# gillesdegottex/percivaltts

Hardware: AMD Instinct MI355X
Metric: acoustic frames/sec per WGAN-GP critic+gen step (higher is better)
Workload: dtype f32

## Files before the change

include/percival_hip.h:

```cpp
#ifndef PERCIVAL_HIP_H
#define PERCIVAL_HIP_H

#include <stddef.h>
#include <stdint.h>

#ifdef __cplusplus
extern "C" {
#endif

#define PTTS_OK            0
#define PTTS_EINVAL       -1
#define PTTS_ELAUNCH      -2
#define PTTS_EWORKSPACE   -3
#define PTTS_EDEVICE      -4

#define PTTS_IN_NONE     0
#define PTTS_IN_LRELU    1
#define PTTS_IN_MASKMUL  2

#define PTTS_PAD_SAME    0
#define PTTS_PAD_CAUSAL  1

#define PTTS_ACT_NONE    0
#define PTTS_ACT_LRELU   1
// ... 79 lines not shown
                          const void* tables, float* partials, size_t partials_bytes, int* nblocks_out, int* npart_out,
                          int B, int T, int F, int L, int cin0, float alpha, void* stream);
int ptts_conv2d_chain_bwd_data(const void* d_last, int d_bf16, const void* maps, const void* a_last, const void* tables,
                               void* gmaps, float* g0, int B, int T, int F, int L, float alpha, void* stream);
int ptts_conv2d_chain_second(const float* u0, const void* gmaps, const void* maps, const void* a_last, const void* tables,
                             void* out, int out_bf16, float* partials, size_t partials_bytes, int* nblocks_out, int* npart_out,
                             int B, int T, int F, int L, int cin0, float alpha, void* stream);

int ptts_gemm(const float* A, const float* Bm, const float* bias, float* C,
              int M, int N, int K,
              int transA, long long lda, long long rows_per_seg, long long seg_stride,
              int transB, long long ldb, long long ldc,
              int in_mode, const float* in_scale, const float* in_shift, const float* mask_src,
              float alpha, int accumulate, const float* out_mask, float* colsum_b, void* stream);

typedef struct ptts_wgrad_desc {
    const float* A; const float* B; float* C; float* colsum_b;
    const float* in_scale; const float* in_shift; const float* mask_src;
    int M, N, K;
    long long lda, ldb, ldc;
    int in_mode; float alpha;
} ptts_wgrad_desc;
int ptts_gemm_wgrad_grouped(const ptts_wgrad_desc* descs, int n, void* stream);

size_t ptts_dense_planes_bytes(int N, int K);
int ptts_split3_dense_weight(const float* w, long long ldw, int K, int N, int transposed, void* planes, void* stream);
typedef struct ptts_dense_split_desc {
    const float* w; void* planes;
    long long ldw;
    int K, N, transposed, reserved;
} ptts_dense_split_desc;
int ptts_split3_dense_weight_grouped(const ptts_dense_split_desc* descs, int n, void* stream);
int ptts_split3_frame_windows(const float* x, int B, int T, int C, int NS, int S, int row_off, int P, int kvalid,
                              void* planes, long long stride_planes_bytes, void* stream);
int ptts_split3_dense_weight_strided(const float* w, long long stride_w, void* planes, long long stride_planes_bytes, int n,
                                     long long ldw, int K, int N, int transposed, void* stream);
int ptts_dense_bf16x6_supported(int M, int N, int K, long long lda, long long ldc);
typedef struct ptts_dense_wgrad_reduce_desc {
    const float* partials;
    int split, Kin, N;
    long long ldc;
    float* C; float* colsum_b;
} ptts_dense_wgrad_reduce_desc;
int ptts_dense_wgrad_bf16x6_supported(int Kin, int N, int M, long long lda, long long ldb);
size_t ptts_dense_wgrad_workspace_bytes(int Kin, int N, int M);
int ptts_dense_wgrad_bf16x6_partials(const float* A, const float* dY, const float* mask_src, const float* in_scale,
                                     const float* in_shift, void* workspace, size_t workspace_bytes, int* split_out,
                                     int Kin, int N, int M, long long lda, long long ldb, int in_mode, float alpha,
                                     void* stream);
int ptts_dense_wgrad_reduce_grouped(const ptts_dense_wgrad_reduce_desc* descs, int n, void* stream);
int ptts_dense_wgrad_bf16x6(const float* A, const float* dY, const float* mask_src, const float* in_scale,
                            const float* in_shift, float* C, float* colsum_b, void* workspace, size_t workspace_bytes,
                            int Kin, int N, int M, long long lda, long long ldb, long long ldc, int in_mode, float alpha,
                            void* stream);
int ptts_dense_bf16x6(const float* A, const void* planes, const float* bias, float* C, int M, int N, int K,
                      long long lda, long long ldc, int in_mode, const float* in_scale, const float* in_shift,
                      const float* mask_src, float alpha, int accumulate, const float* out_mask, void* stream);
int ptts_dense_bf16x6_res(const float* A, const void* planes, const float* bias, float* C, int M, int N, int K,
                          long long lda, long long ldc, int in_mode, const float* in_scale, const float* in_shift,
                          const float* mask_src, float alpha, const float* res, int res_rows, long long ldr,
                          const float* out_mask, void* stream);
int ptts_dense_bf16x6_stats_rows(int M, int N);
int ptts_dense_bf16x6_stats(const float* A, const void* planes, const float* bias, float* C, int M, int N, int K,
                            long long lda, long long ldc, int in_mode, const float* in_scale, const float* in_shift,
                            float alpha, double* stats, int capacity_rows, int* nrows_out, void* stream);
int ptts_dense_bf16x6_bwd_affine(const float* A, const void* planes, float* C, int M, int N, int K, long long lda, long long ldc,
                                 const float* z, const float* scale, const float* shift, float alpha,
                                 double* stats, int capacity_rows, int* nrows_out, void* stream);
int ptts_partial_rows_sum(const double* partials, int nrows, int ncols, double* out, void* stream);
int ptts_dft_mirror(float* Ap, int NB, int B, int Cin, int Kh, void* stream);

int ptts_conv1d_freq_kernel_planes(const float* w, const float* tw, void* planes, int NB, int KW, int Cin, int N, int Kh, void* stream);

int ptts_transpose_batched(const float* src, float* dst, int nb, int rows, int cols, void* stream);
int ptts_conv1d_freq_wgrad_combine(const float* out2, float* dW, int KW, int Cin, int N, int Kh, void* stream);

size_t ptts_conv1d_freq_wgrad_inverse_workspace_bytes(int KW, int Cin, int N);
int ptts_conv1d_freq_wgrad_inverse(const float* Gt, const float* t2, float* dW, void* workspace, size_t workspace_bytes,
                                   int NB, int NBp, int KW, int Cin, int N, int Kh, void* stream);

int ptts_dense_bf16x6_batched(const float* A, long long strideA, const void* planes, long long stride_planes_bytes,
                              const float* bias, float* C, long long strideC, int nbatch, int M, int N, int K,
                              long long lda, long long ldc, int planes_count, void* stream);
int ptts_dense_tn_bf16x6_batched(const float* A, long long strideA, const float* B, long long strideB, float* C, long long strideC,
                                 int nbatch, int M, int Kin, int N, long long lda, long long ldb, long long ldc, int planes_count,
                                 void* stream);

int ptts_split3_frames(const float* x, void* p1, void* p2, void* p3, int B, int T, int C, int pad_left, int pad_right,
                       int Cp, void* stream);
int ptts_split3_weight_t(const float* w, void* p1, void* p2, void* p3, int KW, int C, int N, int Cp, void* stream);
int ptts_conv1d_bf16x6(const void* a1, const void* a2, const void* a3, const void* bt1, const void* bt2, const void* bt3,
                       const float* bias, float* y, int B, int T, int KW, int Cp, int N, void* stream);

int ptts_split3_frames_t(const float* x, void* p1, void* p2, void* p3, int B, int T, int C, int pad_left, int Tp, int Crows,
                         long long Pp, void* stream);
int ptts_conv1d_wgrad_bf16x6(const void* xt1, const void* xt2, const void* xt3, const void* yt1, const void* yt2,
                             const void* yt3, float* dw, int B, int T, int KW, int C, int N, int Crows, long long Pp,
                             void* stream);

int ptts_transpose_frames(const float* x, float* out, int B, int T, int C, int pad_left, int Tp, int Crows, long long Pp,
                          void* stream);
int ptts_conv1d_wgrad_t(const float* xt, const float* yt, float* dw, float* db, int B, int T, int KW, int C, int N, int Crows,
                        long long Pp, void* stream);

size_t ptts_colstats_workspace_bytes(long long rows, int C);
int ptts_colstats(const float* x, long long rows, int C,
                  int in_mode, const float* in_scale, const float* in_shift, const float* mask_src, float alpha,
                  double* sums , void* workspace, size_t workspace_bytes, void* stream);

int ptts_bn_finalize(const double* sums, long long count, const float* gamma, const float* beta,
                     float* moving_mean, float* moving_var, float eps, float momentum,
                     int training, int update_moving, int unbiased_moving, int C,
                     float* scale, float* shift, float* mean , float* rstd , void* stream);

int ptts_bn_batch_stats_supported(long long rows, int C);
int ptts_bn_batch_stats(const float* x, long long rows, int C, const float* gamma, const float* beta,
                        float* moving_mean, float* moving_var, float eps, float momentum, int update_moving, int unbiased_moving,
                        float* scale, float* shift, float* mean , float* rstd ,
                        void* workspace, size_t workspace_bytes, int* counter, void* stream);

int ptts_bn_finalize_partials(const double* partials, int nrows, long long rows, int C, const float* gamma, const float* beta,
                              float* moving_mean, float* moving_var, float eps, float momentum, int update_moving, int unbiased_moving,
                              float* scale, float* shift, float* mean , float* rstd , void* stream);

int ptts_bn_bwd_coefs(const float* dscale, const float* dshift, const float* mean, const float* rstd,
                      const float* gamma , long long count, int C,
                      float* dgamma, float* dbeta, float* c0, float* c2, void* stream);
int ptts_bn_bwd_coefs_acc(const float* dscale, const float* dshift, const float* mean, const float* rstd,
                      const float* gamma , long long count, int C,
                      float* dgamma, float* dbeta, float* c0, float* c2, void* stream);

int ptts_affine_act(const float* x, const float* scale, const float* shift, float* y,
                    long long rows, int C, int act, float alpha, void* stream);
int ptts_affine_act_bwd(const float* dy, const float* x, const float* y, const float* scale, const float* shift,
                        float* dx, double* dsums ,
                        void* workspace, size_t workspace_bytes,
                        long long rows, int C, int act, float alpha, void* stream);
int ptts_gated_mul_fwd(const float* a, const float* b, float* y, long long n, void* stream);
int ptts_gated_mul_bwd(const float* dy, const float* a, const float* b, float* da, float* db, long long n, void* stream);

int ptts_axpby_cols(const float* a, const float* c1, const float* x, const float* c2, const float* c0,
                    float* out, long long rows, int C, void* stream);

int ptts_gp_interpolate(const float* real, const float* fake, const float* alpha_b , float* out,
                        int B, long long TD, void* stream);
int ptts_gp_sqnorm(const float* g, float* out, int B, long long TD, void* stream);
int ptts_gp_penalty(const float* sq , float* penalty , float* coef , int B, void* stream);
int ptts_gp_scale_rows(const float* g, const float* coef, const float* upstream , float* dg,
                       int B, long long TD, void* stream);

int ptts_mean_scaled(const float* v, long long n, float sign, float* out, void* stream);
int ptts_wlse_fwd(const float* y, const float* yhat, const float* w , float* out,
                  long long rows, int D, void* stream);
int ptts_wlse_bwd(const float* y, const float* yhat, const float* w, const float* upstream, float* dyhat,
                  long long rows, int D, void* stream);

int ptts_weight_clip(float* p, long long n, float lo, float hi, void* stream);

int ptts_adam_keras_step(float* p, const float* g, float* m, float* v, long long n,
                         float lr, float b1, float b2, float eps, float gscale,
                         int* step , void* stream);

size_t ptts_lstm_fwd_workspace_bytes(int B, int T, int H, int ndir);
int ptts_lstm_fwd(const float* xproj, const float* U, float* h_out, float* gates, float* c_out,
                  void* workspace, size_t workspace_bytes,
                  int B, int T, int H, int ndir, int reverse, void* stream);
// ... 113 lines not shown
```

percivaltts_amd/csrc/dense.hip:

```cpp
#include "common.h"
#include <cstdlib>

namespace ptts {
namespace dns {

typedef __bf16 bf16x8 __attribute__((ext_vector_type(8)));
typedef __bf16 bf16x4 __attribute__((ext_vector_type(4)));
typedef __bf16 bf16x2 __attribute__((ext_vector_type(2)));
typedef float f32x4 __attribute__((ext_vector_type(4)));
typedef float f32x2 __attribute__((ext_vector_type(2)));
typedef unsigned u32x2 __attribute__((ext_vector_type(2)));
typedef unsigned short u16;

constexpr int THREADS = 512;
constexpr int NBLK = 256;
constexpr int BK = 32;

#define DNS_PRODUCTS(X) X(2, 0) X(1, 1) X(0, 2) X(1, 0) X(0, 1) X(0, 0)
#define DNS_PRODUCTS_NPL(NPL, X) do { if (NPL == 3) { X(2, 0) X(1, 1) X(0, 2) X(1, 0) X(0, 1) } X(0, 0) } while (0)

__device__ __forceinline__ unsigned pk_bf16(float a, float b) {
    return __builtin_bit_cast(unsigned, __builtin_convertvector((f32x2){a, b}, bf16x2));
}
__device__ __forceinline__ void split3_pair(float a, float b, unsigned& p1, unsigned& p2, unsigned& p3) {
// ... 452 lines not shown
                const float gd = v[e] * ((z[e] * osc[e] + osh[e]) > 0.f ? 1.f : g.out_alpha);
                ssum[e] += gd * z[e]; ssq[e] += gd;
                v[e] = gd * osc[e];
            }
        };
        if (interior) {
            f32x4 mk[MT], old[MT];
            if (g.out_mask) {
#pragma unroll
                for (int i = 0; i < MT; ++i) mk[i] = *reinterpret_cast<const f32x4*>(g.out_mask + off0 + (long long)16 * i * g.ldc);
            }
            if (g.res) {
#pragma unroll
                for (int i = 0; i < MT; ++i) old[i] = *reinterpret_cast<const f32x4*>(res_at(m0 + 16 * i + li));
            }
#pragma unroll
            for (int i = 0; i < MT; ++i) {
                f32x4 v = acc[i][j] + bv;
                if (g.om_scale) {
                    aff_store(v, mk[i]);
                } else if (g.out_mask) {
#pragma unroll
                    for (int e = 0; e < 4; ++e) v[e] = v[e] * (mk[i][e] > 0.f ? 1.f : g.out_alpha);
                }
                if (g.res) v += old[i];
                if (g.stats && !g.om_scale) { ssum += v; ssq += v * v; }
                *reinterpret_cast<f32x4*>(g.C + off0 + (long long)16 * i * g.ldc) = v;
            }
        } else {
#pragma unroll
            for (int i = 0; i < MT; ++i) {
                const int m = m0 + 16 * i + li;
                if (m >= g.M) continue;
                const long long off = off0 + (long long)16 * i * g.ldc;
                f32x4 v = acc[i][j] + bv;
                if (g.out_mask) {
                    const f32x4 mk = *reinterpret_cast<const f32x4*>(g.out_mask + off);
                    if (g.om_scale) {
                        aff_store(v, mk);
                    } else {
#pragma unroll
                        for (int e = 0; e < 4; ++e) v[e] = v[e] * (mk[e] > 0.f ? 1.f : g.out_alpha);
                    }
                }
                if (g.res) v += *reinterpret_cast<const f32x4*>(res_at(m));
                if (g.stats && !g.om_scale) { ssum += v; ssq += v * v; }
                *reinterpret_cast<f32x4*>(g.C + off) = v;
            }
        }
        if (g.stats) {
#pragma unroll
            for (int e = 0; e < 4; ++e)
#pragma unroll
                for (int m = 1; m < 16; m <<= 1) { ssum[e] += __shfl_xor(ssum[e], m, 64); ssq[e] += __shfl_xor(ssq[e], m, 64); }
            if (li == 0) {
                double* row = g.stats + (size_t)blockIdx.x * 2 * g.N;
#pragma unroll
                for (int e = 0; e < 4; ++e) { row[n + e] = (double)ssum[e]; row[g.N + n + e] = (double)ssq[e]; }
            }
        }
    }
}

template <int MODE, bool AFFINE, int MT, int NPL>
static void dense_launch_kernel(bool xt, dim3 grid, hipStream_t st, const DenseArgs& g) {
    if constexpr (MT < 8) {
        if (xt) { hipLaunchKernelGGL((dense_bf16x6_kernel<MODE, AFFINE, MT, NPL, true>), grid, dim3(THREADS), 0, st, g); return; }
    }
    hipLaunchKernelGGL((dense_bf16x6_kernel<MODE, AFFINE, MT, NPL>), grid, dim3(THREADS), 0, st, g);
}

static int pick_mt(int M, int col_blocks) {
    static int forced = -1;
    if (forced < 0) { const char* e = getenv("PTTS_DENSE_MT"); forced = e ? atoi(e) : 0; }
    if (forced >= 4 && forced <= 8) return forced;
    int best = 8; double best_eff = -1.0;
    for (int mt = 4; mt <= 8; ++mt) {
        const long long blocks = (long long)((M + 16 * mt - 1) / (16 * mt)) * col_blocks;
        const long long rounds = (blocks + 255) / 256;
        const double eff = (double)M * col_blocks / (double)(rounds * 256 * 16 * mt);
        if (eff > best_eff + 1e-9) { best_eff = eff; best = mt; }
    }
    return best;
}


typedef short s16x4 __attribute__((ext_vector_type(4)));
typedef s16x4 __attribute__((address_space(3)))* lds_s16x4_ptr;
__device__ __forceinline__ bf16x4 tr_read(const u16* p) {
    return __builtin_bit_cast(bf16x4, __builtin_amdgcn_ds_read_tr16_b64_v4i16((lds_s16x4_ptr)(p)));
}
__device__ __forceinline__ bf16x8 cat8(bf16x4 a, bf16x4 b) { return __builtin_shufflevector(a, b, 0, 1, 2, 3, 4, 5, 6, 7); }

struct WgradArgs {
    const float* A; const float* dY; const float* mask_src; const float* in_scale; const float* in_shift;
    float* partials;
    int Kin, N, M;
    long long lda, ldb;
    float alpha;
    int tiles_n, steps_total, split;
    int tiles_k, part;
};

constexpr int WT = 128;
constexpr int WROW = WT;
constexpr int WPL = 32 * WROW;
constexpr int WPART = WT * WT + WT;
constexpr int WXR = 16;
constexpr int WXPL = 32 * WXR + 4 * 64;
constexpr int WPARTX = WXR * WT;
__host__ __device__ inline bool wgrad_has_rem(int Kin) { return Kin > WT && Kin % WT >= 1 && Kin % WT <= WXR; }
__host__ __device__ inline int wgrad_tiles_k(int Kin) { return wgrad_has_rem(Kin) ? Kin / WT : (Kin + WT - 1) / WT; }
__host__ __device__ inline int wgrad_part(int Kin) { return WPART + (wgrad_has_rem(Kin) ? WPARTX : 0); }

template <int MODE, bool AFFINE, int NPL, bool XR = false>
__global__ __launch_bounds__(THREADS) void dense_wgrad_bf16x6_kernel(WgradArgs g) {
    constexpr bool MASK = MODE == PTTS_IN_MASKMUL;
    extern __shared__ __attribute__((aligned(16))) u16 lds_w[];
    const int tid = threadIdx.x, lane = tid & 63;
    const int wave = __builtin_amdgcn_readfirstlane(tid >> 6);
    const int li = lane & 15, lg = lane >> 4;
    const int tile = blockIdx.y, tk = tile / g.tiles_n, tn = tile - tk * g.tiles_n;
    const int k0 = tk * WT, n0 = tn * WT;
    const bool xr_wg = XR && tk == g.tiles_k - 1;
    const int per = (g.steps_total + g.split - 1) / g.split;
    const int s_begin = blockIdx.x * per, s_end = min(g.steps_total, s_begin + per);
    const int nsteps = max(0, s_end - s_begin);

    const int c4 = tid & 31;
    const bool a_ok = k0 + 4 * c4 < g.Kin, d_ok = n0 + 4 * c4 < g.N;
    const float* pa = g.A + (a_ok ? k0 + 4 * c4 : 0);
    const float* pm = MASK ? g.mask_src + (a_ok ? k0 + 4 * c4 : 0) : nullptr;
    const float* pd = g.dY + (d_ok ? n0 + 4 * c4 : 0);
    int dst[2];
#pragma unroll
    for (int j = 0; j < 2; ++j) {
        const int row = (tid + j * THREADS) >> 5;
        dst[j] = row * WROW + ((((c4 >> 2) + row + 4 * (row >> 3)) & 7) << 4) + (c4 & 3) * 4;
    }
    f32x4 sc = {1.f, 1.f, 1.f, 1.f}, sh = {0.f, 0.f, 0.f, 0.f};
    if (AFFINE && a_ok) { sc = *reinterpret_cast<const f32x4*>(g.in_scale + k0 + 4 * c4); sh = *reinterpret_cast<const f32x4*>(g.in_shift + k0 + 4 * c4); }
    const bool xr_stage = xr_wg && wave < 2;
    const int xrow = tid >> 2, xkq = g.tiles_k * WT + 4 * (tid & 3);
    const bool x_ok = xr_stage && xkq < g.Kin;
    const float* pax = g.A + (x_ok ? xkq : 0);
    const float* pmx = MASK ? g.mask_src + (x_ok ? xkq : 0) : nullptr;
    auto xrow_off = [](int row) { return row * WXR + 64 * (row >> 3); };
    const int xdst = xrow_off(xrow & 31) + 4 * (tid & 3);
    f32x4 scx = {1.f, 1.f, 1.f, 1.f}, shx = {0.f, 0.f, 0.f, 0.f};
    if (AFFINE && x_ok) { scx = *reinterpret_cast<const f32x4*>(g.in_scale + xkq); shx = *reinterpret_cast<const f32x4*>(g.in_shift + xkq); }
    struct Stage { f32x4 va[2], vm[MASK ? 2 : 1], vd[2]; bool ok[2]; f32x4 vx, vmx; bool okx; };
    auto load = [&](int s, Stage& sg) {
        if (XR && xr_stage) {
            const int m = (s_begin + s) * 32 + xrow;
            sg.okx = s < nsteps && m < g.M && x_ok;
            const long long r = sg.okx ? m : 0;
            sg.vx = *reinterpret_cast<const f32x4*>(pax + r * g.lda);
            if (MASK) sg.vmx = *reinterpret_cast<const f32x4*>(pmx + r * g.lda);
        }
#pragma unroll
        for (int j = 0; j < 2; ++j) {
            const int m = (s_begin + s) * 32 + ((tid + j * THREADS) >> 5);
            sg.ok[j] = s < nsteps && m < g.M;
            const long long r = sg.ok[j] ? m : 0;
            sg.va[j] = *reinterpret_cast<const f32x4*>(pa + r * g.lda);
            if (MASK) sg.vm[j] = *reinterpret_cast<const f32x4*>(pm + r * g.lda);
// ... 501 lines not shown
static int dense_launch(const float* A, const void* planes, const float* bias, float* C, int M, int N, int K,
                        long long lda, long long ldc, int in_mode, const float* in_scale, const float* in_shift,
                        const float* mask_src, float alpha, const float* res, int res_rows, long long ldr,
                        const float* out_mask, double* stats, int stats_capacity_rows, int* stats_rows_out, void* stream,
                        bool extra_tile) {
    const int accumulate = res != nullptr;
    PTTS_REQUIRE(!res || (res_rows > 0 && ldr >= N && M <= 8LL * res_rows), "dense_bf16x6: bad residual (rows %d, ldr %lld)", res_rows, ldr);
    PTTS_REQUIRE(A && planes && C, "dense_bf16x6: null matrix");
    PTTS_REQUIRE(ptts_dense_bf16x6_supported(M, N, K, lda, ldc), "dense_bf16x6: unsupported shape M=%d N=%d K=%d lda=%lld ldc=%lld (K and lda must be multiples of 4)", M, N, K, lda, ldc);
    PTTS_REQUIRE(lda >= K && ldc >= N, "dense_bf16x6: bad leading dims");
    PTTS_REQUIRE(in_mode >= 0 && in_mode <= 2, "dense_bf16x6: bad in_mode %d", in_mode);
    PTTS_REQUIRE((in_scale == nullptr) == (in_shift == nullptr), "dense_bf16x6: scale/shift must come together");
    PTTS_REQUIRE(in_mode != PTTS_IN_MASKMUL || mask_src, "dense_bf16x6: MASKMUL needs mask_src");
    PTTS_REQUIRE(in_mode == PTTS_IN_LRELU || !in_scale, "dense_bf16x6: scale/shift need PTTS_IN_LRELU");
    PTTS_REQUIRE(!(out_mask && bias), "dense_bf16x6: out_mask with bias is not defined");
    PTTS_REQUIRE(alpha >= 0.f && alpha <= 1.f, "dense_bf16x6: LeakyReLU slope %g outside [0, 1]", alpha);
    const bool vec_out = N % 4 == 0 && ldc % 4 == 0 && ((uintptr_t)C & 15) == 0 && (!bias || ((uintptr_t)bias & 15) == 0) &&
                         (!out_mask || ((uintptr_t)out_mask & 15) == 0) && (!res || (((uintptr_t)res & 15) == 0 && ldr % 4 == 0));
    PTTS_REQUIRE(((uintptr_t)A & 15) == 0 && (!mask_src || ((uintptr_t)mask_src & 15) == 0) &&
                 (!in_scale || (((uintptr_t)in_scale | (uintptr_t)in_shift) & 15) == 0), "dense_bf16x6: A, its mask and scale/shift must be 16-byte aligned");
    DenseArgs g;
    g.A = A; g.mask_src = mask_src; g.in_scale = in_scale; g.in_shift = in_shift; g.planes = (const u16*)planes; g.bias = bias;
    g.out_mask = out_mask; g.C = C; g.M = M; g.N = N; g.K = K;
    g.NT = (N + NBLK - 1) / NBLK * (NBLK / 16); g.KS = (K + BK - 1) / BK;
    g.lda = lda; g.ldc = ldc; g.alpha = alpha; g.out_alpha = alpha; g.accumulate = accumulate; g.has_affine = in_scale != nullptr; g.vec_out = vec_out;
    g.res = res; g.res_rows = res ? res_rows : 1; g.ldr = ldr;
    g.bsA = g.bsP = g.bsC = 0;
    const bool xt = extra_tile && !stats && !g_om_scale && N > NBLK && N % NBLK >= 1 && N % NBLK <= 16;
    const int cb = xt ? N / NBLK : (N + NBLK - 1) / NBLK;
    int mt = pick_mt(M, cb);
    if (xt && mt == 8) mt = 7;
    const dim3 grid((unsigned)((M + 16 * mt - 1) / (16 * mt)), (unsigned)cb);
    g.stats = stats;
    g.om_scale = g_om_scale; g.om_shift = g_om_shift;
    if (stats) {
        PTTS_REQUIRE(vec_out, "dense_bf16x6_stats: N and ldc must be multiples of 4, C (and bias) 16-byte aligned");
        PTTS_REQUIRE(stats_capacity_rows >= (int)grid.x, "dense_bf16x6_stats: room for %d rows of sums, %d needed", stats_capacity_rows, (int)grid.x);
        *stats_rows_out = (int)grid.x;
    }
    hipStream_t st = (hipStream_t)stream;
    const bool one = ptts::bf16_products();
#define DNS_L(MODE, AFF, MT) do { if (one) dense_launch_kernel<MODE, AFF, MT, 1>(xt, grid, st, g); \
                                  else dense_launch_kernel<MODE, AFF, MT, 3>(xt, grid, st, g); } while (0)
#define DNS_M(MT)                                                                \
    do {                                                                         \
        if (in_mode == PTTS_IN_LRELU) { if (in_scale) DNS_L(PTTS_IN_LRELU, true, MT); else DNS_L(PTTS_IN_LRELU, false, MT); } \
        else if (in_mode == PTTS_IN_MASKMUL) DNS_L(PTTS_IN_MASKMUL, false, MT);  \
        else DNS_L(PTTS_IN_NONE, false, MT);                                     \
    } while (0)
    switch (mt) {
        case 4: DNS_M(4); break;
        case 5: DNS_M(5); break;
        case 6: DNS_M(6); break;
        case 7: DNS_M(7); break;
        default: DNS_M(8); break;
    }
#undef DNS_M
#undef DNS_L
    return check_launch("dense_bf16x6");
}

extern "C" int ptts_conv1d_freq_kernel_planes(const float* w, const float* tw, void* planes, int NB, int KW, int Cin, int N, int Kh,
                                              void* stream) {
    PTTS_REQUIRE(w && tw && planes && NB > 0 && Cin > 0 && N > 0, "conv1d_freq_kernel_planes: bad arguments");
    PTTS_REQUIRE(Kh >= Cin && Kh % 8 == 0, "conv1d_freq_kernel_planes: Kh=%d must be a multiple of 8 and >= Cin=%d", Kh, Cin);
    const int NT = (N + NBLK - 1) / NBLK * (NBLK / 16), KS = (2 * Kh + BK - 1) / BK;
    const long long total = (long long)NT * KS * 64;
    const long long fstride = (long long)(ptts_dense_planes_bytes(N, 2 * Kh) / sizeof(u16));
    const dim3 grid((unsigned)((total + 255) / 256), (unsigned)((NB + WDFT_FCH - 1) / WDFT_FCH));
#define WDFT(KWv) hipLaunchKernelGGL(conv1d_wdft_planes_kernel<KWv>, grid, dim3(256), 0, (hipStream_t)stream, w, tw, (u16*)planes, fstride, NB, Cin, N, Kh, NT, KS)
    switch (KW) {
        case 3: WDFT(3); break;
        case 5: WDFT(5); break;
        case 7: WDFT(7); break;
        case 9: WDFT(9); break;
        case 11: WDFT(11); break;
        case 21: WDFT(21); break;
        default: set_error("conv1d_freq_kernel_planes: KW=%d not instantiated (3, 5, 7, 9, 11, 21)", KW); return PTTS_EINVAL;
    }
#undef WDFT
    return check_launch("conv1d_freq_kernel_planes");
}

extern "C" int ptts_dense_bf16x6_batched(const float* A, long long strideA, const void* planes, long long stride_planes_bytes,
                                         const float* bias, float* C, long long strideC, int nbatch, int M, int N, int K,
                                         long long lda, long long ldc, int planes_count, void* stream) {
    PTTS_REQUIRE(A && planes && C && nbatch > 0 && nbatch <= 65535, "dense_bf16x6_batched: bad arguments");
    PTTS_REQUIRE(ptts_dense_bf16x6_supported(M, N, K, lda, ldc), "dense_bf16x6_batched: unsupported shape M=%d N=%d K=%d lda=%lld ldc=%lld", M, N, K, lda, ldc);
    PTTS_REQUIRE(lda >= K && ldc >= N && planes_count >= 1 && planes_count <= 3 && planes_count != 2, "dense_bf16x6_batched: bad leading dims / planes");
    PTTS_REQUIRE(stride_planes_bytes % 16 == 0 && strideA % 4 == 0 && ((uintptr_t)A & 15) == 0, "dense_bf16x6_batched: strides of A / planes must keep 16-byte alignment");
    const bool vec_out = N % 4 == 0 && ldc % 4 == 0 && strideC % 4 == 0 && ((uintptr_t)C & 15) == 0 && (!bias || ((uintptr_t)bias & 15) == 0);
    DenseArgs g;
    g.A = A; g.mask_src = nullptr; g.in_scale = nullptr; g.in_shift = nullptr; g.planes = (const u16*)planes; g.bias = bias;
    g.out_mask = nullptr; g.C = C; g.M = M; g.N = N; g.K = K;
    g.NT = (N + NBLK - 1) / NBLK * (NBLK / 16); g.KS = (K + BK - 1) / BK;
    g.lda = lda; g.ldc = ldc; g.alpha = 0.f; g.out_alpha = 0.f; g.accumulate = 0; g.has_affine = 0; g.vec_out = vec_out;
    g.res = nullptr; g.res_rows = 1; g.ldr = 0;
    g.bsA = strideA; g.bsP = stride_planes_bytes / 2; g.bsC = strideC;
    g.stats = nullptr; g.om_scale = g.om_shift = nullptr;
    const int cb = (N + NBLK - 1) / NBLK;
    int mt = 8; double best_eff = -1.0;
    {
        static int forced = -1;
        if (forced < 0) { const char* e = getenv("PTTS_DENSE_BATCHED_MT"); forced = e ? atoi(e) : 0; }
        for (int m = 8; m >= 4; --m) {
            const int tiles = (M + 16 * m - 1) / (16 * m);
            const double eff = (double)M / (double)(tiles * 16 * m);
            if (eff > best_eff + 1e-9) { best_eff = eff; mt = m; }
        }
        if (forced >= 4 && forced <= 8) mt = forced;
    }
    const dim3 grid((unsigned)((M + 16 * mt - 1) / (16 * mt)), (unsigned)cb, (unsigned)nbatch);
    hipStream_t st = (hipStream_t)stream;
    const bool one = planes_count == 1;
#define DNS_B(MT) do { if (one) hipLaunchKernelGGL((dense_bf16x6_kernel<PTTS_IN_NONE, false, MT, 1>), grid, dim3(THREADS), 0, st, g); \
                       else hipLaunchKernelGGL((dense_bf16x6_kernel<PTTS_IN_NONE, false, MT, 3>), grid, dim3(THREADS), 0, st, g); } while (0)
    switch (mt) {
        case 4: DNS_B(4); break;
        case 5: DNS_B(5); break;
        case 6: DNS_B(6); break;
        case 7: DNS_B(7); break;
        default: DNS_B(8); break;
    }
#undef DNS_B
    return check_launch("dense_bf16x6_batched");
}

extern "C" int ptts_dense_tn_bf16x6_batched(const float* A, long long strideA, const float* B, long long strideB, float* C,
                                            long long strideC, int nbatch, int M, int Kin, int N, long long lda, long long ldb,
                                            long long ldc, int planes_count, void* stream) {
    PTTS_REQUIRE(A && B && C && nbatch > 0 && nbatch <= 65535, "dense_tn_bf16x6_batched: bad arguments");
    PTTS_REQUIRE(M > 0 && Kin > 0 && N > 0, "dense_tn_bf16x6_batched: bad shape M=%d Kin=%d N=%d", M, Kin, N);
    PTTS_REQUIRE(planes_count == 1 || planes_count == 3, "dense_tn_bf16x6_batched: planes_count %d is neither 1 nor 3", planes_count);
    PTTS_REQUIRE(lda >= (Kin + 3) / 4 * 4 && ldb >= (N + 3) / 4 * 4 && ldc >= N, "dense_tn_bf16x6_batched: bad leading dims lda=%lld ldb=%lld ldc=%lld", lda, ldb, ldc);
    PTTS_REQUIRE(strideA >= 0 && strideB >= 0 && strideC >= 0, "dense_tn_bf16x6_batched: negative stride");
    PTTS_REQUIRE(lda % 4 == 0 && ldb % 4 == 0 && ldc % 4 == 0 && strideA % 4 == 0 && strideB % 4 == 0 && strideC % 4 == 0 &&
                 (((uintptr_t)A | (uintptr_t)B | (uintptr_t)C) & 15) == 0, "dense_tn_bf16x6_batched: pointers, leading dims and strides must keep 16-byte alignment");
    TnArgs g;
    g.A = A; g.B = B; g.C = C; g.strideA = strideA; g.strideB = strideB; g.strideC = strideC;
    g.lda = lda; g.ldb = ldb; g.ldc = ldc; g.Kin = Kin; g.N = N; g.M = M;
    g.tiles_n = (N + WT - 1) / WT;
    const long long tiles = (long long)((Kin + WT - 1) / WT) * g.tiles_n;
    PTTS_REQUIRE(tiles <= 0x7fffffffLL, "dense_tn_bf16x6_batched: too many tiles");
    const dim3 grid((unsigned)tiles, 1, (unsigned)nbatch);
    constexpr size_t lds = (size_t)2 * 6 * WPL * sizeof(u16);
    static bool attr = false;
    if (!attr) { (void)hipFuncSetAttribute(reinterpret_cast<const void*>(&dense_tn_bf16x6_kernel<3>), hipFuncAttributeMaxDynamicSharedMemorySize, (int)lds);
                 (void)hipFuncSetAttribute(reinterpret_cast<const void*>(&dense_tn_bf16x6_kernel<1>), hipFuncAttributeMaxDynamicSharedMemorySize, (int)lds); attr = true; }
    if (planes_count == 1) hipLaunchKernelGGL((dense_tn_bf16x6_kernel<1>), grid, dim3(THREADS), lds, (hipStream_t)stream, g);
    else hipLaunchKernelGGL((dense_tn_bf16x6_kernel<3>), grid, dim3(THREADS), lds, (hipStream_t)stream, g);
    return check_launch("dense_tn_bf16x6_batched");
}

extern "C" int ptts_dense_wgrad_bf16x6_supported(int Kin, int N, int M, long long lda, long long ldb) {
    return (Kin > 0 && N > 0 && M > 0 && Kin % 4 == 0 && N % 4 == 0 && lda % 4 == 0 && ldb % 4 == 0 &&
            (long long)wgrad_tiles_k(Kin) * ((N + WT - 1) / WT) <= 65535) ? 1 : 0;
}

namespace {
int wgrad_split(int Kin, int N, int M) {
    const int tiles = wgrad_tiles_k(Kin) * ((N + WT - 1) / WT), steps = (M + 31) / 32;
    int split = (256 + tiles - 1) / tiles;
    static int env_split = -1;
    if (env_split < 0) { const char* e = getenv("PTTS_DENSE_WGRAD_SPLIT"); env_split = e ? atoi(e) : 0; }
    if (env_split > 0) split = env_split;
    if (split > steps) split = steps;
    return split < 1 ? 1 : split;
}
}

extern "C" size_t ptts_dense_wgrad_workspace_bytes(int Kin, int N, int M) {
    if (Kin <= 0 || N <= 0 || M <= 0) return 0;
    const size_t tiles = (size_t)wgrad_tiles_k(Kin) * ((N + WT - 1) / WT);
    return tiles * wgrad_split(Kin, N, M) * wgrad_part(Kin) * sizeof(float);
}

extern "C" int ptts_dense_wgrad_bf16x6_partials(const float* A, const float* dY, const float* mask_src, const float* in_scale,
                                                const float* in_shift, void* workspace, size_t workspace_bytes, int* split_out,
                                                int Kin, int N, int M, long long lda, long long ldb, int in_mode, float alpha,
                                                void* stream) {
    PTTS_REQUIRE(A && dY && workspace && split_out, "dense_wgrad_bf16x6: null pointer");
    PTTS_REQUIRE(ptts_dense_wgrad_bf16x6_supported(Kin, N, M, lda, ldb), "dense_wgrad_bf16x6: unsupported shape Kin=%d N=%d M=%d lda=%lld ldb=%lld", Kin, N, M, lda, ldb);
// ... 82 lines not shown
```

Before: 4.720 million.

## Add persistent LDS-resident kernel for batched dense with shared small A

Adds a persistent kernel for batched dense products where A is shared across the batch (strideA==0, M,K<=128). The kernel splits A into bf16 planes once and keeps them in LDS, then each wave loops over (batch, 32-column slice) items, prefetching the next item's weight planes into registers while computing the current one. It replaces a grid that reloaded and resplit A for every batch and column block, and it launches at most one workgroup per CU. This costs more registers and LDS per workgroup, and parallelism is limited to 8 waves per CU.

```diff
diff --git a/include/percival_hip.h b/include/percival_hip.h
--- a/include/percival_hip.h
+++ b/include/percival_hip.h
@@ -185,6 +185,8 @@
 int ptts_dense_bf16x6_batched(const float* A, long long strideA, const void* planes, long long stride_planes_bytes,
                               const float* bias, float* C, long long strideC, int nbatch, int M, int N, int K,
                               long long lda, long long ldc, int planes_count, void* stream);
+int ptts_set_dense_batched_resident(int on);
+int ptts_dense_batched_resident_eligible(long long strideA, int M, int N, int K, int planes_count);
 int ptts_dense_tn_bf16x6_batched(const float* A, long long strideA, const float* B, long long strideB, float* C, long long strideC,
                                  int nbatch, int M, int Kin, int N, long long lda, long long ldb, long long ldc, int planes_count,
                                  void* stream);
diff --git a/percivaltts_amd/csrc/dense.hip b/percivaltts_amd/csrc/dense.hip
--- a/percivaltts_amd/csrc/dense.hip
+++ b/percivaltts_amd/csrc/dense.hip
@@ -558,6 +558,133 @@
         if (eff > best_eff + 1e-9) { best_eff = eff; best = mt; }
     }
     return best;
+}
+
+constexpr int RES_M = 128, RES_K = 128;
+constexpr int RES_KS = RES_K / BK;
+constexpr int RES_PL = RES_M * BK;
+template <int NPL> constexpr size_t resident_lds_bytes() { return (size_t)RES_KS * NPL * RES_PL * sizeof(u16); }
+
+template <int NPL, int MT = RES_M / 16, int KSC = 0>
+__global__ __launch_bounds__(THREADS) void dense_bf16x6_resident_kernel(DenseArgs g, int slices, int items) {
+    extern __shared__ __attribute__((aligned(16))) u16 lds_r[];
+    const int tid = threadIdx.x, lane = tid & 63;
+    const int wave = __builtin_amdgcn_readfirstlane(tid >> 6);
+    const int li = lane & 15, lg = lane >> 4;
+    const int KS = KSC ? KSC : g.KS;
+    const size_t ps = (size_t)g.NT * KS * 512;
+    const int stride = 8 * (int)gridDim.x;
+    int item = 8 * (int)blockIdx.x + wave;
+    const bool live = item < items;
+
+    constexpr int NQ = RES_M * (RES_K / 4) / THREADS;
+    f32x4 va[NQ];
+#pragma unroll
+    for (int j = 0; j < NQ; ++j) {
+        const int q = tid + j * THREADS, row = q >> 5, k4 = 4 * (q & 31);
+        const bool ok = row < g.M && k4 < g.K;
+        va[j] = *reinterpret_cast<const f32x4*>(g.A + (ok ? (long long)row * g.lda + k4 : 0));
+    }
+
+    bf16x8 wf[RES_KS][2][NPL];
+    auto load_w = [&](int it, int s) {
+        const int z = it / slices, sl = it - z * slices;
+        const u16* wp = g.planes + (long long)z * g.bsP + (((size_t)(2 * sl) * KS + s) * 64 + lane) * 8;
+#pragma unroll
+        for (int j = 0; j < 2; ++j)
+#pragma unroll
+            for (int p = 0; p < NPL; ++p) wf[s][j][p] = *reinterpret_cast<const bf16x8*>(wp + p * ps + (size_t)j * KS * 512);
+    };
+#pragma unroll
+    for (int s = 0; s < RES_KS; ++s) {
+        if (s < KS) load_w(live ? item : items - 1, s);
+        __builtin_amdgcn_sched_barrier(0);
+    }
+
+    {
+#pragma unroll
+        for (int j = 0; j < NQ; ++j) {
+            const int q = tid + j * THREADS, row = q >> 5, s = (q & 31) >> 3, kq = q & 7;
+            u16* d = lds_r + s * NPL * RES_PL + row * BK + ((((kq >> 1) ^ ((row >> 1) & 2))) << 3) + (kq & 1) * 4;
+            const f32x4 a = (row < g.M && 4 * (q & 31) < g.K) ? va[j] : f32x4{0.f, 0.f, 0.f, 0.f};
+            if (NPL == 3) {
+                unsigned a1, a2, a3, b1, b2, b3;
+                split3_pair(a[0], a[1], a1, a2, a3);
+                split3_pair(a[2], a[3], b1, b2, b3);
+                *reinterpret_cast<u32x2*>(d) = (u32x2){a1, b1};
+                *reinterpret_cast<u32x2*>(d + RES_PL) = (u32x2){a2, b2};
+                *reinterpret_cast<u32x2*>(d + 2 * RES_PL) = (u32x2){a3, b3};
+            } else {
+                *reinterpret_cast<u32x2*>(d) = (u32x2){pk_bf16(a[0], a[1]), pk_bf16(a[2], a[3])};
+            }
+        }
+    }
+    __syncthreads();
+    if (!live) return;
+
+    const int boff = li * BK + ((lg ^ ((li >> 1) & 2)) << 3);
+    auto run_item = [&](const int it, const bool has_next, const int next) __attribute__((always_inline)) {
+        const int z = it / slices, sl = it - z * slices;
+        f32x4 bv[2] = {f32x4{0.f, 0.f, 0.f, 0.f}, f32x4{0.f, 0.f, 0.f, 0.f}};
+        if (g.bias) {
+#pragma unroll
+            for (int j = 0; j < 2; ++j)
+#pragma unroll
+                for (int e = 0; e < 4; ++e) bv[j][e] = g.bias[min(32 * sl + 16 * j + 4 * lg + e, g.N - 1)];
+        }
+        f32x4 acc[MT][2];
+#pragma unroll
+        for (int i = 0; i < MT; ++i) { acc[i][0] = f32x4{0.f, 0.f, 0.f, 0.f}; acc[i][1] = f32x4{0.f, 0.f, 0.f, 0.f}; }
+#pragma unroll
+        for (int s = 0; s < RES_KS; ++s) {
+            if (s < KS) {
+                const u16* as = lds_r + s * NPL * RES_PL + boff;
+#pragma unroll
+                for (int i = 0; i < MT; ++i) {
+                    bf16x8 bf[NPL];
+#pragma unroll
+                    for (int p = 0; p < NPL; ++p) bf[p] = *reinterpret_cast<const bf16x8*>(as + p * RES_PL + i * 16 * BK);
+#define DNS_MM(PA, PW)                                                                                    \
+                    acc[i][0] = __builtin_amdgcn_mfma_f32_16x16x32_bf16(wf[s][0][PW < NPL ? PW : 0], bf[PA < NPL ? PA : 0], acc[i][0], 0, 0, 0);    \
+                    acc[i][1] = __builtin_amdgcn_mfma_f32_16x16x32_bf16(wf[s][1][PW < NPL ? PW : 0], bf[PA < NPL ? PA : 0], acc[i][1], 0, 0, 0);
+                    DNS_PRODUCTS_NPL(NPL, DNS_MM);
+#undef DNS_MM
+                }
+                if (has_next) load_w(next, s);
+                if (KSC) __builtin_amdgcn_sched_barrier(0);
+            }
+        }
+        float* __restrict__ Cz = g.C + (long long)z * g.bsC;
+#pragma unroll
+        for (int j = 0; j < 2; ++j) {
+            const int n = 32 * sl + 16 * j + 4 * lg;
+            if (n >= g.N) continue;
+            if (g.vec_out && n + 3 < g.N) {
+#pragma unroll
+                for (int i = 0; i < MT; ++i) {
+                    const int m = 16 * i + li;
+                    if (m < g.M) *reinterpret_cast<f32x4*>(Cz + (long long)m * g.ldc + n) = acc[i][j] + bv[j];
+                }
+            } else {
+#pragma unroll
+                for (int e = 0; e < 4; ++e) {
+                    if (n + e >= g.N) continue;
+#pragma unroll
+                    for (int i = 0; i < MT; ++i) {
+                        const int m = 16 * i + li;
+                        if (m < g.M) Cz[(long long)m * g.ldc + n + e] = acc[i][j][e] + bv[j][e];
+                    }
+                }
+            }
+        }
+    };
+    int next = item + stride;
+    run_item(item, next < items, next);
+    while (next < items) {
+        item = next;
+        next = item + stride;
+        run_item(item, next < items, next);
+    }
 }
 
 
@@ -1225,6 +1352,68 @@
     return check_launch("conv1d_freq_kernel_planes");
 }
 
+static int g_batched_resident = -1;
+static int batched_resident_on() {
+    if (g_batched_resident < 0) { const char* e = getenv("PTTS_DENSE_BATCHED_RESIDENT"); g_batched_resident = e ? (atoi(e) != 0 ? 1 : 0) : 1; }
+    return g_batched_resident;
+}
+extern "C" int ptts_set_dense_batched_resident(int on) {
+    const int prev = batched_resident_on();
+    g_batched_resident = on ? 1 : 0;
+    return prev;
+}
+extern "C" int ptts_dense_batched_resident_eligible(long long strideA, int M, int N, int K, int planes_count) {
+    return (strideA == 0 && M > 0 && M <= RES_M && N > 0 && K > 0 && K <= RES_K && K % 4 == 0 &&
+            (planes_count == 1 || planes_count == 3)) ? 1 : 0;
+}
+
+template <int NPL, int MT>
+static void resident_set_lds() {
+    (void)hipFuncSetAttribute(reinterpret_cast<const void*>(&dense_bf16x6_resident_kernel<NPL, MT, 0>), hipFuncAttributeMaxDynamicSharedMemorySize,
+                              (int)resident_lds_bytes<NPL>());
+    (void)hipFuncSetAttribute(reinterpret_cast<const void*>(&dense_bf16x6_resident_kernel<NPL, MT, RES_KS>), hipFuncAttributeMaxDynamicSharedMemorySize,
+                              (int)resident_lds_bytes<NPL>());
+    if constexpr (MT > 1) resident_set_lds<NPL, MT - 1>();
+}
+static int resident_cus() {
+    constexpr int MAXDEV = 64;
+    static int cus[MAXDEV];
+    int dev = 0;
+    if (hipGetDevice(&dev) != hipSuccess || dev < 0 || dev >= MAXDEV) { set_error("dense_bf16x6_batched: no current device"); return 0; }
+    if (!cus[dev]) {
+        int n = 0;
+        if (hipDeviceGetAttribute(&n, hipDeviceAttributeMultiprocessorCount, dev) != hipSuccess || n <= 0) {
+            set_error("dense_bf16x6_batched: the device does not tell its compute units"); return 0;
+        }
+        resident_set_lds<3, RES_M / 16>();
+        resident_set_lds<1, RES_M / 16>();
+        cus[dev] = n;
+    }
+    return cus[dev];
+}
+static int resident_launch(DenseArgs g, int slices, int items, int planes_count, hipStream_t st) {
+    const int cus = resident_cus();
+    if (!cus) return PTTS_ELAUNCH;
+    const int wgs = (items + 7) / 8;
+    const dim3 grid((unsigned)(wgs < cus ? wgs : cus));
+#define DNS_RK(NPL, MT) do { if (g.KS == RES_KS) hipLaunchKernelGGL((dense_bf16x6_resident_kernel<NPL, MT, RES_KS>), grid, dim3(THREADS), resident_lds_bytes<NPL>(), st, g, slices, items); \
+                             else hipLaunchKernelGGL((dense_bf16x6_resident_kernel<NPL, MT, 0>), grid, dim3(THREADS), resident_lds_bytes<NPL>(), st, g, slices, items); } while (0)
+#define DNS_R(MT) do { if (planes_count == 1) DNS_RK(1, MT); else DNS_RK(3, MT); } while (0)
+    switch ((g.M + 15) / 16) {
+        case 1: DNS_R(1); break;
+        case 2: DNS_R(2); break;
+        case 3: DNS_R(3); break;
+        case 4: DNS_R(4); break;
+        case 5: DNS_R(5); break;
+        case 6: DNS_R(6); break;
+        case 7: DNS_R(7); break;
+        default: DNS_R(8); break;
+    }
+#undef DNS_R
+#undef DNS_RK
+    return check_launch("dense_bf16x6_batched");
+}
+
 extern "C" int ptts_dense_bf16x6_batched(const float* A, long long strideA, const void* planes, long long stride_planes_bytes,
                                          const float* bias, float* C, long long strideC, int nbatch, int M, int N, int K,
                                          long long lda, long long ldc, int planes_count, void* stream) {
@@ -1241,6 +1430,11 @@
     g.res = nullptr; g.res_rows = 1; g.ldr = 0;
     g.bsA = strideA; g.bsP = stride_planes_bytes / 2; g.bsC = strideC;
     g.stats = nullptr; g.om_scale = g.om_shift = nullptr;
+    const long long items = (long long)nbatch * ((N + 31) / 32);
+    if (batched_resident_on() && ptts_dense_batched_resident_eligible(strideA, M, N, K, planes_count) && items <= 0x3fffffffLL) {
+        g.vec_out = ldc % 4 == 0 && strideC % 4 == 0 && ((uintptr_t)C & 15) == 0 && (!bias || ((uintptr_t)bias & 15) == 0);
+        return resident_launch(g, (N + 31) / 32, (int)items, planes_count, (hipStream_t)stream);
+    }
     const int cb = (N + NBLK - 1) / NBLK;
     int mt = 8; double best_eff = -1.0;
     {
```

Measured after the change: 4.794 million, median of 6. 1.02x the previous value.
